# HyeonwooNoh/VQA-Transfer-ExternalData

Measured on AMD Instinct MI355X. Metric: VQA train samples/sec (img+question) at bs512, higher is better.
Workload: dtype f32

## Files before the change

### include/vqa_hot.h

```cpp
#ifndef VQA_HOT_H
#define VQA_HOT_H

#include <stdint.h>

#ifdef __cplusplus
extern "C" {
#endif

#define VQA_HOT_ABI_VERSION 5

enum {
    VQA_OK = 0,
    VQA_ERR_ARG = -1,
    VQA_ERR_ALIGN = -2,
    VQA_ERR_LAUNCH = -3,
    VQA_ERR_UNSUPPORTED = -4,
    VQA_ERR_WORKSPACE = -5
};

int vqa_hot_version(void);
const char* vqa_hot_error_string(int code);

int vqa_gather_features(const float* table, const int32_t* nbox_table, const int64_t* idx,
                        float* V, int32_t* nb, int B, int R, int D, int64_t N, void* stream);

int vqa_embed_fwd(const float* E, const int32_t* q, float* x_tm, int B, int T, int W, int Vq, void* stream);
int vqa_gru_pack_wx(const float* wg, const float* wc, const float* bg, const float* bc, float* wx, float* bx, int W, int H,
                    void* stream);
int vqa_gru_unpack_dwx(const float* dwx, float* gwg, float* gwc, int W, int H, void* stream);
int vqa_embed_fwd_ld(const float* E, const int32_t* q, float* x_tm, int B, int T, int W, int Vq, int ldx, void* stream);
int vqa_gru_unpack_dwx_bias(const float* dwx, float* gwg, float* gwc, float* gbg, float* gbc, int W, int H, void* stream);
int vqa_set_deterministic(int on);
int vqa_embed_bwd(const float* dx_tm, const int32_t* q, float* dE, int B, int T, int W, int Vq, void* stream);
int vqa_embed_bwd_len(const float* dx_tm, const int32_t* q, const int32_t* len, float* dE, int B, int T, int W,
                      int Vq, void* stream);
int vqa_embed_bwd_len_det(const float* dx_tm, const int32_t* q, const int32_t* len, float* dE, int B, int T, int W,
                          int Vq, int deterministic, void* stream);

int vqa_gemm_f32(int transA, int transB, int M, int N, int K, const float* A, int lda, const float* B,
                 int ldb, float* C, int ldc, const float* bias, const float* D, int ldd, int split_k,
                 float* workspace, int64_t workspace_floats, void* stream);
int vqa_gemm_f32_ex(int transA, int transB, int M, int N, int K, const float* A, int lda, const float* B,
                    int ldb, float* C, int ldc, const float* bias, const float* D, int ldd, int split_k,
                    float* workspace, int64_t workspace_floats, int max_blocks, void* stream);
int vqa_gemm_f32_gather(int M, int N, int K, const float* table, int lda, const int64_t* idx, int R,
                        int64_t n_samples_in_table, const float* B, int ldb, float* C, int ldc, const float* bias,
                        float* gathered_out, int ldg, void* stream);
int vqa_gemm_set_max_blocks(int n);
int vqa_gemm_set_order(int order);
int64_t vqa_gemm_workspace_floats(int transA, int transB, int M, int N, int K, int split_k);
int vqa_gemm_set_config(int cfg);
int vqa_gemm_set_gru_config(int cfg);
int vqa_gemm_set_tall_config(int cfg);

int vqa_ln_set_fast(int on);
int vqa_ln_relu_fwd(const float* pre, const float* gamma, const float* beta, const uint8_t* keepmask,
                    float keep_prob, float* y, float* mean, float* rstd, int G, int rows, int N, void* stream);
int vqa_ln_relu_bwd(const float* dy, const float* pre, const float* mean, const float* rstd,
                    const float* gamma, const float* beta, const uint8_t* keepmask, float keep_prob,
                    float* dpre, float* part_dgamma, float* part_dbeta, float* part_dbias, int G, int rows,
                    int N, void* stream);
int vqa_ln_act_fwd(const float* pre, const float* gamma, const float* beta, const uint8_t* keepmask, float keep_prob,
                   float* y, float* mean, float* rstd, int G, int rows, int N, int act, void* stream);
int vqa_ln_act_bwd(const float* dy, const float* pre, const float* mean, const float* rstd, const float* gamma,
                   const float* beta, const uint8_t* keepmask, float keep_prob, float* dpre, float* part_dgamma,
                   float* part_dbeta, float* part_dbias, int G, int rows, int N, int act, void* stream);
int vqa_ln_pair_mul_supported(int N, const void* const* ptrs, int n_ptrs);
int vqa_ln_pair_mul_fwd(const float* pre_a, const float* pre_b, const float* gamma_a, const float* beta_a, const float* gamma_b,
                        const float* beta_b, float* y_a, float* y_b, float* z, float* mean_a, float* rstd_a, float* mean_b,
                        float* rstd_b, int G, int N, void* stream);
int vqa_ln_pair_mul_bwd(const float* dz, const float* add_b, const float* pre_a, const float* pre_b, const float* mean_a,
                        const float* rstd_a, const float* mean_b, const float* rstd_b, const float* gamma_a, const float* beta_a,
                        const float* gamma_b, const float* beta_b, float* dpre_a, float* dpre_b, float* part_dgamma_a,
                        float* part_dbeta_a, float* part_dbias_a, float* part_dgamma_b, float* part_dbeta_b, float* part_dbias_b,
                        int G, int N, void* stream);
int vqa_tanh_fwd(const float* x, float* y, int64_t n, void* stream);
int vqa_tanh_bwd(const float* dy, const float* y, float* dx, int64_t n, void* stream);
int vqa_colsum(const float* X, int M, int N, int ldx, float* out, float* workspace, int64_t workspace_floats,
               void* stream);
int64_t vqa_colsum_workspace_floats(int M, int N);
int vqa_colsum3(const float* X0, const float* X1, const float* X2, int M, int N, int ldx, float* out0, float* out1,
                float* out2, float* workspace, int64_t workspace_floats, void* stream);
int vqa_colsum_acc(const float* X, int M, int N, int ldx, float* out, int accumulate, float* workspace,
                   int64_t workspace_floats, void* stream);
int vqa_colsum3_acc(const float* X0, const float* X1, const float* X2, int M, int N, int ldx, float* out0, float* out1,
                    float* out2, int acc_mask, float* workspace, int64_t workspace_floats, void* stream);
int vqa_mul(const float* a, const float* b, float* z, int64_t n, void* stream);
int vqa_mul_bwd(const float* dz, const float* a, const float* b, float* da, float* db, int64_t n, void* stream);
int vqa_add_inplace(float* acc, const float* x, int64_t n, void* stream);

int vqa_gru_gates_fwd(const float* gpre, int ldg, const float* h_prev, float* r, float* u, float* rh, int B,
                      int H, void* stream);
int vqa_gru_cand_fwd(const float* cpre, int ldc, const float* u, const float* h_prev, const int32_t* len, int t,
                     float* c, float* h_new, int B, int H, void* stream);
int vqa_gru_bwd_a(const float* dh, const float* h_prev, const float* u, const float* c, const int32_t* len,
                  int t, float* dc_pre, int ld_dc, float* du_pre, int ld_du, float* dh_acc, int B, int H,
                  void* stream);
int vqa_gru_bwd_b(const float* drh, const float* h_prev, const float* r, float* dr_pre, int ld_dr,
                  float* dh_acc, int B, int H, void* stream);

int vqa_gru_seq_fwd(float* xp, const float* Wg_h, const float* Wc_h, const int32_t* len, float* hs, float* r,
                    float* u, float* c, float* rh, int T, int B, int H, void* stream);
int vqa_gru_seq_bwd(float* dh_T, const float* Wg_h, const float* Wc_h, const int32_t* len, const float* hs,
                    const float* r, const float* u, const float* c, float* dxp, float* dh_scratch, int T, int B,
                    int H, void* stream);

int vqa_gru_seq_fwd_live(float* xp, const float* Wg_h, const float* Wc_h, const int32_t* len, const int32_t* live_rows,
                         float* hs, float* r, float* u, float* c, float* rh, int T, int B, int H, void* stream);
int vqa_gru_seq_bwd_live(float* dh_T, const float* Wg_h, const float* Wc_h, const int32_t* len,
                         const int32_t* live_rows, const float* hs, const float* r, const float* u, const float* c,
                         float* dxp, float* dh_scratch, int T, int B, int H, void* stream);
int vqa_gru_fill_finished(float* hs, float* rh, const int32_t* len, int T, int B, int H, void* stream);
int vqa_gru_zero_finished(float* dxp, const int32_t* len, int T, int B, int H, void* stream);

int vqa_gru_seq_fwd_persistent(const float* xp, const float* Wg_h, const float* Wc_h, const int32_t* len, float* hs,
                               float* r, float* u, float* c, float* rh, int T, int B, int H, unsigned* sync,
                               void* stream);
int vqa_gru_fwd_persistent_supported(int T, int B, int H);
int64_t vqa_gru_persistent_sync_bytes(void);
int vqa_gru_set_persistent(int mode);
int vqa_gru_persistent_set_census(unsigned* dev_words);

int vqa_gru_seq_fwd_ws(const float* xp, const float* Wg_h, const float* Wc_h, const int32_t* len, float* hs, float* r,
                       float* u, float* c, float* rh, int T, int B, int H, void* ws, void* stream);
int vqa_gru_ws_supported(int T, int B, int H);
int vqa_gru_seq_bwd_ws(const float* dh_T, const float* d_outs, const float* Wg_h, const float* Wc_h, const int32_t* len,
                       const float* hs, const float* r, const float* u, const float* c, float* dxp, int T, int B, int H,
                       void* ws, void* stream);
int vqa_gru_ws_bwd_supported(int T, int B, int H);
int64_t vqa_gru_ws_workspace_bytes(int T);
int vqa_gru_ws_set_mode(int mode);
int vqa_gru_ws_set_form(int form);
int vqa_gru_ws_set_stamps(unsigned long long* dev_words);

int vqa_gru_seq_fwd_rows(float* xp, const float* Wg_h, const float* Wc_h, const int32_t* len, float* hs, float* r,
                         float* u, float* c, float* rh, int T, int B, int H, int row0, int rows, void* stream);
// ... 338 lines not shown
```

### vqa-transfer-externaldata_amd/_lib.py

```python
from __future__ import annotations

import ctypes as C
import os

_HERE = os.path.dirname(os.path.abspath(__file__))
_LIB_PATH = os.path.join(_HERE, "libvqahot.so")


class VqaHotError(RuntimeError):
    pass


def lib_path():
    return _LIB_PATH


class Dims(C.Structure):
    _fields_ = [("B", C.c_int32), ("R", C.c_int32), ("D", C.c_int32), ("H", C.c_int32), ("T", C.c_int32),
                ("W", C.c_int32), ("A", C.c_int32), ("Vq", C.c_int32), ("N_img", C.c_int64),
                ("model_type", C.c_int32), ("keep_att", C.c_float), ("keep_joint", C.c_float),
                ("inv_global_batch", C.c_float), ("flags", C.c_int32),
                ("num_marginal", C.c_int32), ("ent_cols", C.c_int32), ("extra_weight", C.c_float),
                ("map_dim", C.c_int32), ("La", C.c_int32)]

# ... 24 lines not shown
    _fields_ = [("table", C.c_void_p), ("nbox_table", C.c_void_p), ("image_idx", C.c_void_p),
                ("q_intseq", C.c_void_p), ("q_intseq_len", C.c_void_p), ("answer_target", C.c_void_p),
                ("train_mask", C.c_void_p), ("obj_mask", C.c_void_p), ("attr_mask", C.c_void_p),
                ("exist_mask", C.c_void_p), ("keep_att", C.c_void_p), ("keep_joint", C.c_void_p),
                ("keep_joint2", C.c_void_p), ("live_rows", C.c_void_p), ("noise", C.c_void_p), ("keep_tile", C.c_void_p),
                ("keep_word", C.c_void_p), ("answer_intseq", C.c_void_p), ("answer_intseq_len", C.c_void_p)]


class PtDims(C.Structure):
    _fields_ = [(k, C.c_int32) for k in ("B", "n", "R", "D", "H", "W", "A", "Vq", "n_ws", "L", "flags")] + \
               [("keep_att", C.c_float), ("keep_joint", C.c_float), ("global_valid", C.c_float * 2)]


class PtFc(C.Structure):
    _fields_ = [("w", C.c_void_p), ("b", C.c_void_p), ("beta", C.c_void_p * 4), ("gamma", C.c_void_p * 4)]


class PtParams(C.Structure):
    _fields_ = [("wordset_map", C.c_void_p), ("l_glove", C.c_void_p), ("spat_v_linear_v", PtFc),
                ("spat_q_linear_v", PtFc), ("spat_att_score", PtFc), ("gru_wg", C.c_void_p), ("gru_bg", C.c_void_p),
                ("gru_wc", C.c_void_p), ("gru_bc", C.c_void_p), ("pooled_linear_l", PtFc), ("q_linear_l", PtFc),
                ("joint_fc", PtFc), ("wordset_ft", PtFc), ("classifier", PtFc)]


class PtKind(C.Structure):
    _fields_ = [(k, C.c_void_p) for k in ("normal_boxes", "fills", "blanks", "blanks_len", "wordsets", "num", "keep_att",
                                          "keep_bf_joint", "keep_ws_joint")]


class PtBatch(C.Structure):
    _fields_ = [("image_ft", C.c_void_p), ("spatial_ft", C.c_void_p), ("num_boxes", C.c_void_p), ("kind", PtKind * 2),
                ("perm", C.c_void_p), ("inv", C.c_void_p), ("live_rows", C.c_void_p)]


PT_HEAD_BF, PT_HEAD_WS, PT_HEAD_EW = 1, 2, 4


class PtExtDims(C.Structure):
    _fields_ = [("base", PtDims), ("heads", C.c_int32), ("Lc", C.c_int32), ("n_ctx", C.c_int32)]


class PtFc6(C.Structure):
    _fields_ = [("w", C.c_void_p), ("b", C.c_void_p), ("beta", C.c_void_p * 6), ("gamma", C.c_void_p * 6)]


class PtExtParams(C.Structure):
    _fields_ = [("wordset_map", C.c_void_p), ("l_glove", C.c_void_p), ("enwiki_map", C.c_void_p),
                ("spat_v_linear_v", PtFc6), ("spat_q_linear_v", PtFc6), ("spat_att_score", PtFc6)] + \
               [(k, C.c_void_p) for k in ("gru_wg", "gru_bg", "gru_wc", "gru_bc", "egru_wg", "egru_bg", "egru_wc",
                                          "egru_bc")] + \
               [(k, PtFc6) for k in ("pooled_linear_l", "q_linear_l", "joint_fc", "wordset_ft", "classifier")]


class PtCtxKind(C.Structure):
    _fields_ = [(k, C.c_void_p) for k in ("context", "context_len", "keep_ew_joint")]


class PtExtBatch(C.Structure):
    _fields_ = [("base", PtBatch), ("ctx", PtCtxKind * 2), ("ctx_perm", C.c_void_p), ("ctx_inv", C.c_void_p),
                ("ctx_live_rows", C.c_void_p)]


_P, _I, _L, _F = C.c_void_p, C.c_int, C.c_int64, C.c_float

SIGNATURES = {
    "vqa_hot_version": (_I, []),
    "vqa_hot_error_string": (C.c_char_p, [_I]),
    "vqa_gather_features": (_I, [_P, _P, _P, _P, _P, _I, _I, _I, _L, _P]),
    "vqa_embed_fwd": (_I, [_P, _P, _P, _I, _I, _I, _I, _P]),
    "vqa_gru_pack_wx": (_I, [_P, _P, _P, _P, _P, _P, _I, _I, _P]),
    "vqa_gru_unpack_dwx": (_I, [_P, _P, _P, _I, _I, _P]),
    "vqa_embed_fwd_ld": (_I, [_P, _P, _P, _I, _I, _I, _I, _I, _P]),
    "vqa_gru_unpack_dwx_bias": (_I, [_P, _P, _P, _P, _P, _I, _I, _P]),
    "vqa_embed_bwd": (_I, [_P, _P, _P, _I, _I, _I, _I, _P]),
    "vqa_embed_bwd_len": (_I, [_P, _P, _P, _P, _I, _I, _I, _I, _P]),
    "vqa_embed_bwd_len_det": (_I, [_P, _P, _P, _P, _I, _I, _I, _I, _I, _P]),
    "vqa_set_deterministic": (_I, [_I]),
    "vqa_gemm_f32": (_I, [_I, _I, _I, _I, _I, _P, _I, _P, _I, _P, _I, _P, _P, _I, _I, _P, _L, _P]),
    "vqa_gemm_workspace_floats": (_L, [_I, _I, _I, _I, _I, _I]),
    "vqa_gemm_f32_ex": (_I, [_I, _I, _I, _I, _I, _P, _I, _P, _I, _P, _I, _P, _P, _I, _I, _P, _L, _I, _P]),
    "vqa_gemm_f32_gather": (_I, [_I, _I, _I, _P, _I, _P, _I, _L, _P, _I, _P, _I, _P, _P, _I, _P]),
    "vqa_gemm_set_tall_config": (_I, [_I]),
    "vqa_gemm_set_max_blocks": (_I, [_I]),
    "vqa_gemm_set_order": (_I, [_I]),
    "vqa_gemm_set_config": (_I, [_I]),
    "vqa_conv_set_config": (_I, [_I]),
    "vqa_gemm_set_gru_config": (_I, [_I]),
    "vqa_gru_seq_fwd": (_I, [_P, _P, _P, _P, _P, _P, _P, _P, _P, _I, _I, _I, _P]),
    "vqa_gru_seq_fwd_persistent": (_I, [_P, _P, _P, _P, _P, _P, _P, _P, _P, _I, _I, _I, _P, _P]),
    "vqa_gru_fwd_persistent_supported": (_I, [_I, _I, _I]),
    "vqa_gru_persistent_sync_bytes": (_L, []),
    "vqa_gru_set_persistent": (_I, [_I]),
    "vqa_gru_persistent_set_census": (_I, [_P]),
    "vqa_gru_seq_fwd_ws": (_I, [_P, _P, _P, _P, _P, _P, _P, _P, _P, _I, _I, _I, _P, _P]),
    "vqa_gru_ws_supported": (_I, [_I, _I, _I]),
    "vqa_gru_seq_bwd_ws": (_I, [_P, _P, _P, _P, _P, _P, _P, _P, _P, _P, _I, _I, _I, _P, _P]),
    "vqa_gru_ws_bwd_supported": (_I, [_I, _I, _I]),
    "vqa_gru_ws_workspace_bytes": (_L, [_I]),
    "vqa_gru_ws_set_mode": (_I, [_I]),
    "vqa_gru_ws_set_form": (_I, [_I]),
    "vqa_gru_ws_set_stamps": (_I, [_P]),
    "vqa_gru_seq_fwd_rows": (_I, [_P, _P, _P, _P, _P, _P, _P, _P, _P, _I, _I, _I, _I, _I, _P]),
    "vqa_gru_seq_bwd_rows": (_I, [_P, _P, _P, _P, _P, _P, _P, _P, _P, _P, _I, _I, _I, _I, _I, _P]),
    "vqa_gru_seq_bwd": (_I, [_P, _P, _P, _P, _P, _P, _P, _P, _P, _P, _I, _I, _I, _P]),
    "vqa_gru_seq_fwd_live": (_I, [_P, _P, _P, _P, _P, _P, _P, _P, _P, _P, _I, _I, _I, _P]),
    "vqa_gru_seq_bwd_live": (_I, [_P, _P, _P, _P, _P, _P, _P, _P, _P, _P, _P, _I, _I, _I, _P]),
    "vqa_gru_fill_finished": (_I, [_P, _P, _P, _I, _I, _I, _P]),
    "vqa_gru_zero_finished": (_I, [_P, _P, _I, _I, _I, _P]),
    "vqa_ln_set_fast": (_I, [_I]),
    "vqa_ln_relu_fwd": (_I, [_P, _P, _P, _P, _F, _P, _P, _P, _I, _I, _I, _P]),
    "vqa_ln_relu_bwd": (_I, [_P, _P, _P, _P, _P, _P, _P, _F, _P, _P, _P, _P, _I, _I, _I, _P]),
    "vqa_ln_act_fwd": (_I, [_P, _P, _P, _P, _F, _P, _P, _P, _I, _I, _I, _I, _P]),
    "vqa_ln_act_bwd": (_I, [_P, _P, _P, _P, _P, _P, _P, _F, _P, _P, _P, _P, _I, _I, _I, _I, _P]),
    "vqa_ln_pair_mul_supported": (_I, [_I, _P, _I]),
    "vqa_ln_pair_mul_fwd": (_I, [_P] * 13 + [_I, _I, _P]),
    "vqa_ln_pair_mul_bwd": (_I, [_P] * 20 + [_I, _I, _P]),
    "vqa_tanh_fwd": (_I, [_P, _P, _L, _P]),
    "vqa_tanh_bwd": (_I, [_P, _P, _P, _L, _P]),
    "vqa_softmax_ce_fwd": (_I, [_P, _P, _P, _I, _P, _P, _P, _I, _I, _P]),
    "vqa_softmax_set_fast": (_I, [_I]),
    "vqa_colsum": (_I, [_P, _I, _I, _I, _P, _P, _L, _P]),
    "vqa_colsum_workspace_floats": (_L, [_I, _I]),
    "vqa_colsum3": (_I, [_P, _P, _P, _I, _I, _I, _P, _P, _P, _P, _L, _P]),
    "vqa_colsum_acc": (_I, [_P, _I, _I, _I, _P, _I, _P, _L, _P]),
    "vqa_colsum3_acc": (_I, [_P, _P, _P, _I, _I, _I, _P, _P, _P, _I, _P, _L, _P]),
    "vqa_mul": (_I, [_P, _P, _P, _L, _P]),
    "vqa_mul_bwd": (_I, [_P, _P, _P, _P, _P, _L, _P]),
    "vqa_add_inplace": (_I, [_P, _P, _L, _P]),
    "vqa_gru_gates_fwd": (_I, [_P, _I, _P, _P, _P, _P, _I, _I, _P]),
    "vqa_gru_cand_fwd": (_I, [_P, _I, _P, _P, _P, _I, _P, _P, _I, _I, _P]),
    "vqa_gru_bwd_a": (_I, [_P, _P, _P, _P, _P, _I, _P, _I, _P, _I, _P, _I, _I, _P]),
    "vqa_gru_bwd_b": (_I, [_P, _P, _P, _P, _I, _P, _I, _I, _P]),
    "vqa_attn_set_fast": (_I, [_I]),
    "vqa_attn_pool_fwd": (_I, [_P, _P, _P, _P, _P, _P, _P, _F, _P, _P, _I, _I, _I, _I, _P]),
    "vqa_attn_pool_bwd": (_I, [_P, _P, _P, _P, _P, _P, _P, _F, _P, _P, _P, _P, _I, _I, _I, _I, _P]),
    "vqa_attn_pool_fwd_rep": (_I, [_P, _P, _P, _P, _P, _P, _P, _F, _P, _P, _I, _I, _I, _I, _I, _P]),
    "vqa_attn_pool_bwd_rep": (_I, [_P, _P, _P, _P, _P, _P, _P, _F, _P, _P, _P, _P, _I, _I, _I, _I, _I, _P]),
    "vqa_loss_fwd": (_I, [_P, _P, _P, _P, _P, _P, _I, _F, _P, _P, _P, _I, _I, _P]),
    "vqa_loss2_fwd": (_I, [_P, _P, _P, _P, _P, _P, _P, _F, _P, _P, _P, _P, _P, _I, _I, _I, _P]),
    "vqa_rowmin_mask_fwd": (_I, [_P, _P, _P, _P, _I, _I, _P]),
    "vqa_rowmin_mask_bwd": (_I, [_P, _P, _P, _P, _I, _I, _P]),
    "vqa_report_reduce": (_I, [_P, _I, _P, _P]),
    "vqa_report_key": (C.c_char_p, [_I]),
    "vqa_sumsq": (_I, [_P, _L, _P, _P, _P, _L, _P]),
    "vqa_sumsq_workspace_floats": (_L, [_L]),
    "vqa_clip_adam": (_I, [_P, _P, _P, _P, _L, _P, _F, _F, _F, _F, _F, _P]),
    "vqa_dropout_mask": (_I, [_P, _L, C.c_uint64, C.c_uint64, _F, _P]),
    "vqa_clip_adam_dev": (_I, [_P, _P, _P, _P, _L, _P, _F, _P, _F, _F, _F, _P]),
    "vqa_embed2_fwd": (_I, [_P, _P, _P, _P, _I, _I, _I, _I, _P]),
    "vqa_embed2_bwd": (_I, [_P, _P, _P, _P, _I, _I, _I, _I, _P]),
    "vqa_lstm_step_fwd": (_I, [_P, _P, _P, _P, _I, _P, _P, _I, _I, _P]),
    "vqa_lstm_step_bwd": (_I, [_P, _P, _P, _P, _P, _P, _I, _P, _P, _P, _I, _I, _P]),
    "vqa_relu_fwd": (_I, [_P, _P, _L, _P]),
    "vqa_relu_bwd": (_I, [_P, _P, _P, _L, _P]),
    "vqa_fill": (_I, [_P, _L, _F, _P]),
    "vqa_score_fwd": (_I, [_P, _P, _P, _P, _P, _I, _I, _I, _P]),
    "vqa_score_bwd": (_I, [_P, _P, _P, _P, _P, _P, _P, _I, _I, _I, _P]),
    "vqa_reverse_tokens": (_I, [_P, _P, _P, _I, _I, _P]),
    "vqa_bi_outputs_fwd": (_I, [_P, _P, _P, _P, _P, _I, _I, _I, _P]),
    "vqa_bi_outputs_bwd": (_I, [_P, _P, _P, _P, _P, _P, _P, _I, _I, _I, _P]),
    "vqa_bi_dx_combine": (_I, [_P, _P, _P, _P, _I, _I, _I, _P]),
    "vqa_gru_seq_bwd_outs": (_I, [_P, _P, _P, _P, _P, _P, _P, _P, _P, _P, _P, _I, _I, _I, _P]),
    "vqa_adam_lr_step": (_I, [_P, _P, C.c_double, C.c_double, _P, _P]),
    "vqa_graph_capture_begin": (_I, [_P]),
    "vqa_graph_capture_end": (_I, [_P, C.POINTER(C.c_void_p), C.POINTER(C.c_int)]),
    "vqa_graph_capture_abort": (_I, [_P]),
# ... 93 lines not shown
```

### vqa-transfer-externaldata_amd/csrc/gemm_f32.hip

```cpp

#include "vqa_common.h"
#include "gemm_args.h"
#include <cstdio>
#include <cstdlib>

#ifndef VQA_GEMM_STAGGER
#define VQA_GEMM_STAGGER 1
#endif

typedef float f32x16 __attribute__((ext_vector_type(16)));
typedef unsigned int u32x4 __attribute__((ext_vector_type(4)));

#if defined(VQA_DBG_STAMPS)
__device__ unsigned long long* g_dbg_stamps = nullptr;
#define DBG_STAMP(i) do { if (threadIdx.x == 0) dbg_t[i] = __builtin_amdgcn_s_memrealtime(); } while (0)
#else
#define DBG_STAMP(i) do {} while (0)
#endif

namespace {


__device__ __forceinline__ int xcd_remap(int lin, int total) {
    const int q = total >> 3, r = total & 7;
// ... 843 lines not shown
        a.m_fastest = (g_force_order >= 0) ? g_force_order : (m_fast < n_fast ? 1 : 0);
    }
    a.vec_epi = (a.N % 4 == 0) && (a.ldc % 4 == 0) && vqa_aligned16(a.C) && (a.slab_stride % 4 == 0) &&
                (a.D == nullptr || (a.ldd % 4 == 0 && vqa_aligned16(a.D))) &&
                (a.bias == nullptr || vqa_aligned16(a.bias)) && (a.scale == nullptr || vqa_aligned16(a.scale));
    int blocks = a.tiles_m * a.tiles_n * split;
    if (max_blocks > 0 && WGK == 1 && EPI == EPI_PLAIN && blocks > max_blocks) blocks = max_blocks;
    hipLaunchKernelGGL(kern, dim3(blocks), dim3(NT), lds, st, a, ep);
    VQA_CHECK_LAUNCH();
    return VQA_OK;
}

template <int BM, int BN, int WM, int WN, int WGK, int BK, int DEEP, int NT = 256>
int launch_cfg(int tA, int tB, const GemmArgs& a, int split, hipStream_t st, int mb) {
    const EpiArgs ep{};
    if (tA == 0 && tB == 0)
        return launch_one<BM, BN, WM, WN, WGK, BK, DEEP, true, false, EPI_PLAIN, false, false, NT>(a, ep, split, st, mb);
    if (tA == 0 && tB == 1)
        return launch_one<BM, BN, WM, WN, WGK, BK, DEEP, true, true, EPI_PLAIN, false, false, NT>(a, ep, split, st, mb);
    return launch_one<BM, BN, WM, WN, WGK, BK, DEEP, false, false, EPI_PLAIN, false, false, NT>(a, ep, split, st, mb);
}

struct TileCfg { int BM, BN; };
constexpr int NUM_CFG = 24;
const TileCfg kCfg[NUM_CFG] = {{128, 128}, {128, 128}, {64, 64}, {64, 64}, {64, 64}, {128, 64}, {64, 128},
                               {64, 32}, {32, 32}, {32, 64}, {64, 64}, {64, 32}, {64, 64}, {64, 32}, {128, 32},
                               {128, 64}, {128, 128}, {128, 128}, {256, 64}, {128, 128}, {128, 64}, {64, 128}, {128, 64}, {64, 32}};

bool fast_ok(int tA, int tB, GemmArgs& a) {
    if (!a.vecA || !a.vecB || a.K < 4 || (a.K % 4) != 0) return false;
    if (tA && ((a.M % 4) != 0 || a.M < 4)) return false;
    if (!tB && ((a.N % 4) != 0 || a.N < 4)) return false;
    const int64_t ab = (tA ? ((int64_t)(a.K - 1) * a.lda + a.M) : ((int64_t)(a.M - 1) * a.lda + a.K)) * 4;
    const int64_t bb = (tB ? ((int64_t)(a.N - 1) * a.ldb + a.K) : ((int64_t)(a.K - 1) * a.ldb + a.N)) * 4;
    if (ab >= 0xFFFFFF00ll || bb >= 0xFFFFFF00ll) return false;
    a.a_bytes = (unsigned)ab;
    a.b_bytes = (unsigned)bb;
    return true;
}

int launch_edge(int tA, int tB, const GemmArgs& a, int split, hipStream_t st) {
    const EpiArgs ep{};
    if (tA == 0 && tB == 0)
        return launch_one<64, 64, 32, 32, 1, 16, false, true, false, EPI_PLAIN, false, true>(a, ep, split, st, 0);
    if (tA == 0 && tB == 1)
        return launch_one<64, 64, 32, 32, 1, 16, false, true, true, EPI_PLAIN, false, true>(a, ep, split, st, 0);
    return launch_one<64, 64, 32, 32, 1, 16, false, false, false, EPI_PLAIN, false, true>(a, ep, split, st, 0);
}

int launch_by_id(int cfg, int tA, int tB, const GemmArgs& a_in, int split, hipStream_t st, int mb = 0) {
    GemmArgs a = a_in;
    if (!fast_ok(tA, tB, a)) return launch_edge(tA, tB, a, split, st);
    switch (cfg) {
        case 0: return launch_cfg<128, 128, 64, 64, 1, 16, false>(tA, tB, a, split, st, mb);
        case 1: return launch_cfg<128, 128, 64, 64, 1, 32, false>(tA, tB, a, split, st, mb);
        case 2: return launch_cfg<64, 64, 32, 32, 1, 16, false>(tA, tB, a, split, st, mb);
        case 3: return launch_cfg<64, 64, 32, 32, 1, 32, false>(tA, tB, a, split, st, mb);
        case 4: return launch_cfg<64, 64, 32, 32, 1, 64, false>(tA, tB, a, split, st, mb);
        case 5: return launch_cfg<128, 64, 64, 32, 1, 32, false>(tA, tB, a, split, st, mb);
        case 6: return launch_cfg<64, 128, 32, 64, 1, 32, false>(tA, tB, a, split, st, mb);
        case 7: return launch_cfg<64, 32, 32, 32, 2, 64, false>(tA, tB, a, split, st, mb);
        case 8: return launch_cfg<32, 32, 32, 32, 4, 64, false>(tA, tB, a, split, st, mb);
        case 9: return launch_cfg<32, 64, 32, 32, 2, 64, false>(tA, tB, a, split, st, mb);
        case 10: return launch_cfg<64, 64, 32, 32, 1, 64, true>(tA, tB, a, split, st, mb);
        case 11: return launch_cfg<64, 32, 32, 32, 2, 64, true>(tA, tB, a, split, st, mb);
        case 12: return launch_cfg<64, 64, 32, 32, 1, 32, true>(tA, tB, a, split, st, mb);
        case 13: return launch_cfg<64, 32, 32, 32, 2, 32, true>(tA, tB, a, split, st, mb);
        case 14: return launch_cfg<128, 32, 32, 32, 1, 64, true>(tA, tB, a, split, st, mb);
        case 15: return launch_cfg<128, 64, 32, 64, 1, 32, true>(tA, tB, a, split, st, mb);
        case 16: return launch_cfg<128, 128, 64, 32, 1, 32, 0, 512>(tA, tB, a, split, st, mb);
        case 17: return launch_cfg<128, 128, 32, 64, 1, 32, 0, 512>(tA, tB, a, split, st, mb);
        case 18: return launch_cfg<256, 64, 64, 32, 1, 32, 0, 512>(tA, tB, a, split, st, mb);
        case 19: return launch_cfg<128, 128, 64, 32, 1, 16, 0, 512>(tA, tB, a, split, st, mb);
        case 20: return launch_cfg<128, 64, 32, 32, 1, 32, 0, 512>(tA, tB, a, split, st, mb);
        case 21: return launch_cfg<64, 128, 32, 32, 1, 32, 0, 512>(tA, tB, a, split, st, mb);
        case 22: return launch_cfg<128, 64, 32, 32, 1, 16, 0, 512>(tA, tB, a, split, st, mb);
        case 23: return launch_cfg<64, 32, 32, 32, 4, 32, 1, 512>(tA, tB, a, split, st, mb);
        default: return VQA_ERR_ARG;
    }
}

}
int vqa_gru_rs_launch(int epi, const GemmArgs& a, const EpiArgs& ep, hipStream_t st);
namespace {
template <int EPI>
int launch_gru(int cfg, const GemmArgs& a_in, const EpiArgs& ep, hipStream_t st) {
    constexpr bool BKC = (EPI == EPI_BWD_RH || EPI == EPI_BWD_DH);
    GemmArgs a = a_in;
    if (!fast_ok(0, BKC ? 1 : 0, a)) return VQA_ERR_ALIGN;
    if (cfg == 30) {
        const int rc = vqa_gru_rs_launch(EPI, a_in, ep, st);
        if (rc != VQA_ERR_UNSUPPORTED) return rc;
        cfg = 16;
    }
    switch (cfg) {
        case 4: return launch_one<64, 64, 32, 32, 1, 64, false, true, BKC, EPI>(a, ep, 1, st);
        case 7: return launch_one<64, 32, 32, 32, 2, 64, false, true, BKC, EPI>(a, ep, 1, st);
        case 8: return launch_one<32, 32, 32, 32, 4, 64, false, true, BKC, EPI>(a, ep, 1, st);
        case 9: return launch_one<32, 64, 32, 32, 2, 64, false, true, BKC, EPI>(a, ep, 1, st);
        case 10: return launch_one<64, 64, 32, 32, 1, 64, true, true, BKC, EPI>(a, ep, 1, st);
        case 11: return launch_one<64, 32, 32, 32, 2, 64, true, true, BKC, EPI>(a, ep, 1, st);
        case 12: return launch_one<64, 64, 32, 32, 1, 32, true, true, BKC, EPI>(a, ep, 1, st);
        case 13: return launch_one<64, 32, 32, 32, 2, 32, true, true, BKC, EPI>(a, ep, 1, st);
        case 16: return launch_one<32, 32, 32, 32, 4, 32, true, true, BKC, EPI>(a, ep, 1, st);
        case 20: return launch_one<128, 64, 32, 32, 1, 32, 0, true, BKC, EPI, false, false, 512>(a, ep, 1, st);
        case 21: return launch_one<64, 128, 32, 32, 1, 32, 0, true, BKC, EPI, false, false, 512>(a, ep, 1, st);
        case 17: return launch_one<64, 32, 32, 32, 4, 32, 1, true, BKC, EPI, false, false, 512>(a, ep, 1, st);
        case 18:
            if (EPI == EPI_GATES) return launch_one<64, 64, 32, 32, 4, 64, 1, true, BKC, EPI, false, false, 1024>(a, ep, 1, st);
            return launch_one<64, 32, 32, 32, 8, 64, 1, true, BKC, EPI, false, false, 1024>(a, ep, 1, st);
        default: return VQA_ERR_ARG;
    }
}

inline int64_t cdiv(int64_t a, int64_t b) { return (a + b - 1) / b; }

int g_force_cfg = -1;
int g_tall_cfg = 20;
int g_max_blocks = 0;
int g_conv_cfg = -1;
int g_conv_cfg_plain = -1;
int g_gru_cfg = -1;
inline int env_cfg(const char* name, int dflt) {
    const char* e = getenv(name);
    return e ? atoi(e) : dflt;
}
inline int gru_cfg_fwd(int rows) {
    static const int mid = env_cfg("VQA_HOT_GRU_MID_FWD", 9), tall = env_cfg("VQA_HOT_GRU_TALL_FWD", 12);
    return g_gru_cfg >= 0 ? g_gru_cfg : (rows >= 2048 ? tall : rows > 512 ? mid : rows > 256 ? 18 : 16);
}
inline int gru_narrow_override() {
    static const int v = [] { const char* e = getenv("VQA_HOT_GRU_NARROW_CFG"); return e ? atoi(e) : 9; }();
    return v;
}
inline int gru_cfg_fwd_cand(int rows) {
    return (g_gru_cfg < 0 && rows >= 2048 && gru_narrow_override() >= 0) ? gru_narrow_override() : gru_cfg_fwd(rows);
}
inline int gru_cfg_bwd(int rows) {
    static const int mid = env_cfg("VQA_HOT_GRU_MID_BWD", 17), tall = env_cfg("VQA_HOT_GRU_TALL_BWD", 13);
    return g_gru_cfg >= 0 ? g_gru_cfg : (rows >= 2048 ? tall : rows > 512 ? mid : rows > 256 ? 18 : 16);
}

inline int tall_small_cfg() {
    static const int v = [] { const char* e = getenv("VQA_HOT_TALL_SMALL_CFG"); return e ? atoi(e) : 12; }();
    return v < NUM_CFG ? v : 12;
}

inline int tune_pair(const char* env, int cfg, int split) {
    const char* e = getenv(env);
    if (e != nullptr) {
        int c = 0, s = 0;
        if (sscanf(e, "%d:%d", &c, &s) == 2 && c >= 0 && c < NUM_CFG && s >= 0 && s <= 16) { cfg = c; split = s; }
    }
    return (cfg << 8) | split;
}

void choose(int tA, int tB, int M, int N, int K, int& cfg, int& split) {
    int64_t target;
    if (tA) {
        static const int tn_short = env_cfg("VQA_HOT_TN_SHORT_CFG", 20);
        static const int tn_mid = env_cfg("VQA_HOT_TN_MID_CFG", 20);
        const bool mid = K < 20000 && cdiv(M, 128) * cdiv(N, 128) <= 128;
        cfg = ((int64_t)M * N >= (1 << 20)) ? (K <= 4096 ? tn_short : (mid ? tn_mid : 19)) : 3;
        target = 512;
    }
    else if (M >= 2048) {
        cfg = (N >= 512) ? (K >= 2048 ? g_tall_cfg : 22) : 13;
        target = 256;
        if (N >= 512 && cdiv(M, 128) * cdiv(N, 64) < 1024 && tall_small_cfg() >= 0) cfg = tall_small_cfg();
    }
    else { cfg = (!tB && N > 2048) ? 13 : 23; target = 256; }
    int want_split = 0;
    if (!tA && tB && M >= 4096 && N <= 320 && K >= 2048) {
        static const int t = tune_pair("VQA_HOT_DX_TUNE", 3, 4);
        if (t >> 8) { cfg = t >> 8; want_split = t & 255; }
    } else if (tA && M <= 320 && N >= 2048 && K >= 4096) {
        static const int t = tune_pair("VQA_HOT_DWX_TUNE", 21, 4);
        if (t >> 8) { cfg = t >> 8; want_split = t & 255; }
    }
    if (g_force_cfg >= 0 && g_force_cfg < NUM_CFG) { cfg = g_force_cfg; want_split = 0; }
    const int64_t blocks = cdiv(M, kCfg[cfg].BM) * cdiv(N, kCfg[cfg].BN);
    if (split <= 0) {
        split = 1;
        if ((N % 4) == 0) {
            if (want_split > 0) split = want_split;
            else
                while (blocks * split < target && K / (split * 2) >= 256 && split < 16) split *= 2;
        }
    }
}

GemmArgs make_args(int M, int N, int K, const float* A, int lda, const float* B, int ldb, float* C, int ldc,
                   const float* bias, const float* D, int ldd) {
    GemmArgs a;
    a.M = M; a.N = N; a.K = K;
    a.A = A; a.lda = lda; a.B = B; a.ldb = ldb; a.C = C; a.ldc = ldc;
    a.bias = bias; a.D = D; a.ldd = ldd;
    a.vecA = (lda % 4 == 0) && vqa_aligned16(A);
    a.vecB = (ldb % 4 == 0) && vqa_aligned16(B);
    a.slab_stride = 0;
    a.k_per_split = (int)cdiv(std::max(K, 1), 64) * 64;
    a.scale = nullptr; a.relu = 0;
    a.a_bytes = a.b_bytes = 0;
    a.Hi = a.Wi = a.Ci = a.Ho = a.Wo = a.cstride = a.pad_t = a.pad_l = a.kw = a.conv_taps = 0;
    a.g_idx = nullptr; a.g_R = 1; a.g_N = 0; a.g_out = nullptr; a.g_ldo = 0;
    return a;
}

}

extern "C" int64_t vqa_gemm_workspace_floats(int transA, int transB, int M, int N, int K, int split_k) {
    int cfg, split = split_k;
    choose(transA, transB, M, N, K, cfg, split);
    return split > 1 ? (int64_t)split * M * N : 0;
}

extern "C" int vqa_gemm_set_config(int cfg) {
    VQA_REQUIRE(cfg >= -1 && cfg < NUM_CFG, VQA_ERR_ARG);
    g_force_cfg = cfg;
    return VQA_OK;
}

extern "C" int vqa_gemm_set_gru_config(int cfg) {
    VQA_REQUIRE(cfg == -1 || cfg == 4 || (cfg >= 7 && cfg <= 13) || (cfg >= 16 && cfg <= 18) || cfg == 20 || cfg == 21 || cfg == 30,
                VQA_ERR_ARG);
    g_gru_cfg = cfg;
    return VQA_OK;
}

int g_shortk_mode = -1;
inline int shortk_mode() {
    if (g_shortk_mode < 0) {
        const char* e = getenv("VQA_HOT_SHORTK");
        g_shortk_mode = e ? (atoi(e) & 3) : 3;
    }
    return g_shortk_mode;
}
int g_bf16x3_mode = -1;
inline int bf16x3_mode() {
    if (g_bf16x3_mode < 0) {
        const char* e = getenv("VQA_HOT_BF16X3");
        g_bf16x3_mode = (e && atoi(e) != 0) ? 1 : 0;
    }
    return g_bf16x3_mode;
}
extern "C" int vqa_gemm_bf16x3_set_mode(int on) {
    g_bf16x3_mode = on < 0 ? -1 : (on ? 1 : 0);
    return VQA_OK;
}
extern "C" int vqa_gemm_shortk_set_mode(int mode) {
    g_shortk_mode = mode < 0 ? -1 : (mode & 3);
    return VQA_OK;
}

extern "C" int vqa_gemm_f32(int transA, int transB, int M, int N, int K, const float* A, int lda, const float* B,
                            int ldb, float* C, int ldc, const float* bias, const float* D, int ldd, int split_k,
                            float* workspace, int64_t workspace_floats, void* stream) {
    return vqa_gemm_f32_ex(transA, transB, M, N, K, A, lda, B, ldb, C, ldc, bias, D, ldd, split_k, workspace,
                           workspace_floats, g_max_blocks, stream);
}

#if defined(VQA_DBG_STAMPS)
extern "C" int vqa_gemm_dbg_stamps(void* buf) {
    unsigned long long* b = static_cast<unsigned long long*>(buf);
    return hipMemcpyToSymbol(HIP_SYMBOL(g_dbg_stamps), &b, sizeof(b)) == hipSuccess ? VQA_OK : VQA_ERR_LAUNCH;
}
#endif

extern "C" int vqa_gemm_set_order(int order) {
    g_force_order = (order == 0 || order == 1) ? order : -1;
    return VQA_OK;
}

extern "C" int vqa_gemm_set_max_blocks(int n) {
    g_max_blocks = n > 0 ? n : 0;
    return VQA_OK;
}

extern "C" int vqa_gemm_f32_ex(int transA, int transB, int M, int N, int K, const float* A, int lda, const float* B,
                               int ldb, float* C, int ldc, const float* bias, const float* D, int ldd, int split_k,
                               float* workspace, int64_t workspace_floats, int max_blocks, void* stream) {
    VQA_REQUIRE(M >= 0 && N >= 0 && K >= 0, VQA_ERR_ARG);
    if (M == 0 || N == 0) return VQA_OK;
    VQA_REQUIRE(A && B && C, VQA_ERR_ARG);
    VQA_REQUIRE(!(transA == 1 && transB == 1), VQA_ERR_UNSUPPORTED);
    VQA_REQUIRE(lda >= (transA ? M : K) && ldb >= (transB ? K : N) && ldc >= N, VQA_ERR_ARG);
    VQA_REQUIRE(D == nullptr || ldd >= N, VQA_ERR_ARG);
    hipStream_t st = static_cast<hipStream_t>(stream);

    if (bf16x3_mode() && !transB && D == nullptr && max_blocks == 0 && g_force_cfg < 0 && vqa_gemm_bf16x3_supported(M, N, K) &&
        (int64_t)M * N * K >= (1ll << 32) && lda % 4 == 0 && ldb % 4 == 0 && vqa_aligned16(A) && vqa_aligned16(B)) {
        const int tiles = (M / 128) * (N / 128);
        int sp = 1;
        while (tiles * sp < 256 && K / (sp * 2) >= 512 && sp < 16) sp *= 2;
        while (sp > 1 && (workspace == nullptr || workspace_floats < (int64_t)sp * M * N || ldc % 4 != 0 || !vqa_aligned16(C))) sp /= 2;
        return vqa_gemm_bf16x3(transA, M, N, K, A, lda, B, ldb, C, ldc, bias, sp, workspace, workspace_floats, stream);
    }
    if (!transA && !transB && split_k <= 1 && max_blocks == 0 && g_force_cfg < 0 && (shortk_mode() & 1) &&
        M >= 1024 && K <= 304 && vqa_gemm_shortk_supported(M, N, K, lda, ldb, ldc) && !(K > 256 && D != nullptr) && vqa_aligned16(A) &&
        vqa_aligned16(B))
        return vqa_gemm_shortk_nn(M, N, K, A, lda, B, ldb, C, ldc, bias, nullptr, D, ldd, 0, stream);

    int cfg, split = split_k;
    choose(transA, transB, M, N, K, cfg, split);
    if (split > 1 && ((N % 4) != 0 || workspace == nullptr)) split = 1;

    GemmArgs a = make_args(M, N, K, A, lda, B, ldb, C, ldc, bias, D, ldd);
    if (split > 1) {
        VQA_REQUIRE(workspace_floats >= (int64_t)split * M * N, VQA_ERR_WORKSPACE);
        int kps = (int)cdiv(cdiv(K, split), 64) * 64;
        a.k_per_split = kps;
        split = (int)cdiv(K, kps);
    }
    if (split > 1) {
        a.C = workspace; a.ldc = N; a.slab_stride = (int64_t)M * N;
        int rc = launch_by_id(cfg, transA, transB, a, split, st, max_blocks);
        if (rc != VQA_OK) return rc;
        const int64_t n4 = (int64_t)M * N / 4;
        const int grid = (int)std::min<int64_t>(cdiv(n4, 256), 2048);
        hipLaunchKernelGGL(splitk_reduce_kernel, dim3(grid), dim3(256), 0, st, workspace, C, M, N, ldc, split);
        VQA_CHECK_LAUNCH();
        return VQA_OK;
    }
    a.k_per_split = (int)cdiv(std::max(K, 1), 64) * 64;
    return launch_by_id(cfg, transA, transB, a, 1, st, max_blocks);
}

extern "C" int vqa_gemm_f32_gather(int M, int N, int K, const float* table, int lda, const int64_t* idx, int R,
                                   int64_t n_samples_in_table, const float* B, int ldb, float* C, int ldc,
                                   const float* bias, float* gathered_out, int ldg, void* stream) {
    VQA_REQUIRE(M >= 0 && N >= 0 && K > 0 && R > 0 && n_samples_in_table > 0, VQA_ERR_ARG);
    if (M == 0 || N == 0) return VQA_OK;
    VQA_REQUIRE(table && idx && B && C, VQA_ERR_ARG);
    VQA_REQUIRE(lda >= K && ldb >= N && ldc >= N && (gathered_out == nullptr || ldg >= K), VQA_ERR_ARG);
    VQA_REQUIRE(K % 32 == 0 && N % 4 == 0, VQA_ERR_UNSUPPORTED);
    VQA_REQUIRE(lda % 4 == 0 && vqa_aligned16(table) && ldb % 4 == 0 && vqa_aligned16(B) &&
                    (gathered_out == nullptr || (ldg % 4 == 0 && vqa_aligned16(gathered_out))),
                VQA_ERR_ALIGN);
    GemmArgs a = make_args(M, N, K, table, lda, B, ldb, C, ldc, bias, nullptr, 0);
    const int64_t bb = ((int64_t)(K - 1) * ldb + N) * 4;
    VQA_REQUIRE(bb < 0xFFFFFF00ll, VQA_ERR_UNSUPPORTED);
    a.a_bytes = 0;
    a.b_bytes = (unsigned)bb;
    VQA_REQUIRE(gathered_out == nullptr || ((int64_t)(M - 1) * ldg + K) * 4 < 0xFFFFFF00ll, VQA_ERR_UNSUPPORTED);
    a.g_idx = idx; a.g_R = R; a.g_N = n_samples_in_table; a.g_out = gathered_out; a.g_ldo = ldg;
    a.k_per_split = (int)cdiv(K, 64) * 64;
    const EpiArgs ep{};
    hipStream_t st = static_cast<hipStream_t>(stream);
    if (g_tall_cfg == 21)
        return launch_one<64, 128, 32, 32, 1, 32, 0, true, false, EPI_PLAIN, false, false, 512, true>(a, ep, 1, st, 0);
    return launch_one<128, 64, 32, 32, 1, 32, 0, true, false, EPI_PLAIN, false, false, 512, true>(a, ep, 1, st, 0);
}

extern "C" int vqa_gemm_set_tall_config(int cfg) {
    VQA_REQUIRE(cfg == 20 || cfg == 21, VQA_ERR_ARG);
    g_tall_cfg = cfg;
    return VQA_OK;
}

extern "C" int vqa_gru_seq_fwd(float* xp, const float* Wg_h, const float* Wc_h, const int32_t* len, float* hs,
                               float* r, float* u, float* c, float* rh, int T, int B, int H, void* stream) {
    return vqa_gru_seq_fwd_rows(xp, Wg_h, Wc_h, len, hs, r, u, c, rh, T, B, H, 0, B, stream);
}

extern "C" int vqa_gru_seq_fwd_rows(float* xp, const float* Wg_h, const float* Wc_h, const int32_t* len, float* hs,
                                    float* r, float* u, float* c, float* rh, int T, int B, int H, int row0, int rows,
                                    void* stream) {
    VQA_REQUIRE(xp && Wg_h && Wc_h && len && hs && r && u && c && rh && T >= 0 && B > 0 && H > 0, VQA_ERR_ARG);
    VQA_REQUIRE(row0 >= 0 && rows >= 0 && row0 + rows <= B, VQA_ERR_ARG);
    VQA_REQUIRE(H % 4 == 0, VQA_ERR_ALIGN);
    if (rows == 0) return VQA_OK;
    hipStream_t st = static_cast<hipStream_t>(stream);
    const int64_t BH = (int64_t)B * H, o = (int64_t)row0 * H;
    for (int t = 0; t < T; ++t) {
        float* xpt = xp + ((int64_t)t * B + row0) * 3 * H;
        const float* hp = hs + t * BH + o;
        EpiArgs eg{};
        eg.H = H; eg.h_prev = hp; eg.o0 = r + t * BH + o; eg.o1 = u + t * BH + o; eg.o2 = rh + t * BH + o;
        GemmArgs ag = make_args(rows, 2 * H, H, hp, H, Wg_h, 2 * H, nullptr, 0, nullptr, xpt, 3 * H);
        int rc = launch_gru<EPI_GATES>(gru_cfg_fwd(rows), ag, eg, st);
        if (rc != VQA_OK) return rc;
        EpiArgs ec{};
        ec.H = H; ec.t = t; ec.len = len + row0; ec.h_prev = hp; ec.i0 = u + t * BH + o; ec.o0 = c + t * BH + o;
        ec.o1 = hs + (t + 1) * BH + o;
        GemmArgs ac = make_args(rows, H, H, rh + t * BH + o, H, Wc_h, H, nullptr, 0, nullptr, xpt + 2 * H, 3 * H);
        rc = launch_gru<EPI_CAND>(gru_cfg_fwd_cand(rows), ac, ec, st);
        if (rc != VQA_OK) return rc;
    }
    return VQA_OK;
}

extern "C" int vqa_gru_seq_fwd_live(float* xp, const float* Wg_h, const float* Wc_h, const int32_t* len,
                                    const int32_t* live_rows, float* hs, float* r, float* u, float* c, float* rh,
                                    int T, int B, int H, void* stream) {
    VQA_REQUIRE(xp && Wg_h && Wc_h && len && live_rows && hs && r && u && c && rh && T >= 0 && B > 0 && H > 0, VQA_ERR_ARG);
// ... 223 lines not shown
```

Measured before the change: 159,500.

## Add batch-sized GEMM kernel with intra-block K split and LDS reduction

Adds a new 512-thread, 64xBN tile GEMM kernel. Its waves split the K dimension inside the block and reduce partial sums through LDS, so no split-K workspace pass or separate reduce kernel is needed. It is routed by default for specific shapes: config 23 with M of 256 to 512 and N up to 1024, and transA split-2 config 20 cases. The aim is to raise per-tile parallelism for mid-sized batch GEMMs and drop the extra reduction launch. The trade-off is one block per CU with heavy LDS use, plus a new code path whose numerics differ in summation order.

After: 160,100 (median of 6 runs). No clear change (+0.4%).

```diff
diff --git a/include/vqa_hot.h b/include/vqa_hot.h
--- a/include/vqa_hot.h
+++ b/include/vqa_hot.h
@@ -52,6 +52,7 @@
 int vqa_gemm_set_config(int cfg);
 int vqa_gemm_set_gru_config(int cfg);
 int vqa_gemm_set_tall_config(int cfg);
+int vqa_gemm_batch_set_mode(int mode);
 
 int vqa_ln_set_fast(int on);
 int vqa_ln_relu_fwd(const float* pre, const float* gamma, const float* beta, const uint8_t* keepmask,
diff --git a/vqa-transfer-externaldata_amd/_lib.py b/vqa-transfer-externaldata_amd/_lib.py
--- a/vqa-transfer-externaldata_amd/_lib.py
+++ b/vqa-transfer-externaldata_amd/_lib.py
@@ -130,6 +130,7 @@
     "vqa_gemm_f32_gather": (_I, [_I, _I, _I, _P, _I, _P, _I, _L, _P, _I, _P, _I, _P, _P, _I, _P]),
     "vqa_gemm_set_tall_config": (_I, [_I]),
     "vqa_gemm_set_max_blocks": (_I, [_I]),
+    "vqa_gemm_batch_set_mode": (_I, [_I]),
     "vqa_gemm_set_order": (_I, [_I]),
     "vqa_gemm_set_config": (_I, [_I]),
     "vqa_conv_set_config": (_I, [_I]),
diff --git a/vqa-transfer-externaldata_amd/csrc/gemm_batch.hip b/vqa-transfer-externaldata_amd/csrc/gemm_batch.hip
--- /dev/null
+++ b/vqa-transfer-externaldata_amd/csrc/gemm_batch.hip
@@ -0,0 +1,280 @@
+
+#include "vqa_common.h"
+#include "gemm_args.h"
+
+namespace {
+
+typedef float f32x16 __attribute__((ext_vector_type(16)));
+typedef unsigned int u32x4 __attribute__((ext_vector_type(4)));
+
+constexpr int BM = 64;
+constexpr int NT = 512;
+constexpr unsigned OOB = 0xFFFFFFF0u;
+
+__device__ __forceinline__ int xcd_remap(int lin, int total) {
+    const int q = total >> 3, r = total & 7;
+    const int xcd = lin & 7, idx = lin >> 3;
+    return (xcd < r ? xcd * (q + 1) : r * (q + 1) + (xcd - r) * q) + idx;
+}
+
+__device__ __forceinline__ float4 as_f4(u32x4 v) {
+    return make_float4(__uint_as_float(v.x), __uint_as_float(v.y), __uint_as_float(v.z), __uint_as_float(v.w));
+}
+
+template <int BR, int DEPTH, bool KC, bool HALVES>
+struct Tile {
+    static constexpr int LD = DEPTH + 4;
+    static constexpr int FL = KC ? BR * LD : DEPTH * BR;
+    static constexpr int QPR = KC ? DEPTH / 4 : BR / 4;
+    static constexpr int NV = BR * DEPTH / 4 / NT;
+    static_assert(NV * NT == BR * DEPTH / 4, "whole float4 per thread");
+    unsigned off[NV];
+    u32x4 reg[NV];
+
+    __device__ __forceinline__ void init(int ld, int r0, int RLIM, int kadd) {
+#pragma unroll
+        for (int i = 0; i < NV; ++i) {
+            const int idx = threadIdx.x + i * NT;
+            const int a = idx / QPR, q = (idx % QPR) * 4;
+            if (KC) {
+                const int k = (HALVES && q >= DEPTH / 2) ? q + kadd : q;
+                off[i] = (unsigned)(((int64_t)min(r0 + a, RLIM - 1) * ld + k) * 4);
+            } else {
+                const int k = (HALVES && a >= DEPTH / 2) ? a + kadd : a;
+                off[i] = (unsigned)(((int64_t)k * ld + (r0 + q < RLIM ? r0 + q : 0)) * 4);
+            }
+        }
+    }
+    __device__ __forceinline__ void load(__amdgpu_buffer_rsrc_t rs, unsigned soff) {
+#pragma unroll
+        for (int i = 0; i < NV; ++i) reg[i] = __builtin_amdgcn_raw_buffer_load_b128(rs, off[i], soff, 0);
+    }
+    __device__ __forceinline__ void load_tail(__amdgpu_buffer_rsrc_t rs, int ld, int k0, int K) {
+#pragma unroll
+        for (int i = 0; i < NV; ++i) {
+            const int idx = threadIdx.x + i * NT;
+            const int a = idx / QPR, q = (idx % QPR) * 4;
+            const int k = k0 + (KC ? q : a);
+            const unsigned kb = (unsigned)(KC ? k0 : k0 * ld) * 4u;
+            reg[i] = __builtin_amdgcn_raw_buffer_load_b128(rs, k < K ? off[i] + kb : OOB, 0, 0);
+        }
+    }
+    __device__ __forceinline__ void store(float* s) const {
+#pragma unroll
+        for (int i = 0; i < NV; ++i) {
+            const int idx = threadIdx.x + i * NT;
+            const int a = idx / QPR, q = (idx % QPR) * 4;
+            *reinterpret_cast<float4*>(s + a * (KC ? LD : BR) + q) = as_f4(reg[i]);
+        }
+    }
+};
+
+template <int BR, int DEPTH, bool KC>
+__device__ __forceinline__ float4 frag4(const float* s, int r0, int c, int lane) {
+    const int i = lane & 31, h = lane >> 5;
+    if (KC) return *reinterpret_cast<const float4*>(s + (r0 + i) * (DEPTH + 4) + c * 8 + h * 4);
+    const float* p = s + (c * 8 + h * 4) * BR + r0 + i;
+    return make_float4(p[0], p[BR], p[2 * BR], p[3 * BR]);
+}
+
+template <bool HALVES>
+struct Form {
+    static constexpr int TN = HALVES ? 2 : 1;
+    static constexpr int BN = 32 * TN;
+    static constexpr int G = HALVES ? 2 : 4;
+    static constexpr int SUB = 8 / G;
+    static constexpr int SUB_N = SUB / 2;
+    static constexpr int TW = TN / SUB_N;
+    static constexpr int DEPTH = 128;
+    static constexpr int STEP = HALVES ? DEPTH / 2 : DEPTH;
+    static constexpr int NC = DEPTH / 8 / G;
+};
+
+template <bool HALVES, bool A_KC, bool B_KC>
+constexpr size_t lds_bytes() {
+    using F = Form<HALVES>;
+    const size_t a = A_KC ? BM * (F::DEPTH + 4) : F::DEPTH * BM, b = B_KC ? F::BN * (F::DEPTH + 4) : F::DEPTH * F::BN;
+    const size_t ops = 2 * (a + b), red = (size_t)F::G * BM * (F::BN + 4);
+    return (ops > red ? ops : red) * sizeof(float);
+}
+
+template <bool HALVES, bool A_KC, bool B_KC>
+__global__ __launch_bounds__(NT, 1) void gemm_batch_kernel(GemmArgs p) {
+    using F = Form<HALVES>;
+    constexpr int BN = F::BN, G = F::G, SUB = F::SUB, TW = F::TW, DEPTH = F::DEPTH, NC = F::NC;
+    using TA = Tile<BM, DEPTH, A_KC, HALVES>;
+    using TB = Tile<BN, DEPTH, B_KC, HALVES>;
+    extern __shared__ __attribute__((aligned(16))) float smem[];
+    float* const L0 = smem;
+    float* const L1 = smem + TA::FL + TB::FL;
+
+    const int lane = threadIdx.x & 63, wave = threadIdx.x >> 6;
+    const int sub = wave % SUB, g = wave / SUB;
+    const int wr = (sub & 1) * 32, wc = (sub >> 1) * TW * 32;
+    const int tile = xcd_remap(blockIdx.x, p.tiles_m * p.tiles_n);
+    const int m0 = (tile % p.tiles_m) * BM, n0 = (tile / p.tiles_m) * BN;
+
+    f32x16 acc[TW];
+#pragma unroll
+    for (int b = 0; b < TW; ++b)
+#pragma unroll
+        for (int r = 0; r < 16; ++r) acc[b][r] = 0.f;
+
+    const __amdgpu_buffer_rsrc_t rsA = __builtin_amdgcn_make_buffer_rsrc(const_cast<float*>(p.A), 0, (int)p.a_bytes, 0x00020000);
+    const __amdgpu_buffer_rsrc_t rsB = __builtin_amdgcn_make_buffer_rsrc(const_cast<float*>(p.B), 0, (int)p.b_bytes, 0x00020000);
+    const int kadd = p.k_per_split - F::STEP;
+    TA sa;
+    TB sb;
+    sa.init(p.lda, m0, p.M, kadd);
+    sb.init(p.ldb, n0, p.N, kadd);
+    const unsigned stepA = (unsigned)(A_KC ? F::STEP : F::STEP * p.lda) * 4u;
+    const unsigned stepB = (unsigned)(B_KC ? F::STEP : F::STEP * p.ldb) * 4u;
+    const int nfull = HALVES ? p.k_per_split / F::STEP : p.K / DEPTH;
+    const int nt = HALVES ? nfull : nfull + (p.K % DEPTH != 0);
+    auto fetch = [&](int t) {
+        if (HALVES || t < nfull) {
+            sa.load(rsA, (unsigned)t * stepA);
+            sb.load(rsB, (unsigned)t * stepB);
+        } else {
+            sa.load_tail(rsA, p.lda, t * DEPTH, p.K);
+            sb.load_tail(rsB, p.ldb, t * DEPTH, p.K);
+        }
+    };
+    auto chunk = [&](int cc) { return HALVES ? g * NC + cc : cc * G + g; };
+    auto compute = [&](const float* As, const float* Bs) {
+        float4 af[2], bf[2][TW];
+        af[0] = frag4<BM, DEPTH, A_KC>(As, wr, chunk(0), lane);
+#pragma unroll
+        for (int b = 0; b < TW; ++b) bf[0][b] = frag4<BN, DEPTH, B_KC>(Bs, wc + b * 32, chunk(0), lane);
+#pragma unroll
+        for (int cc = 0; cc < NC; ++cc) {
+            const int cur = cc & 1, nx = cur ^ 1;
+            if (cc + 1 < NC) {
+                af[nx] = frag4<BM, DEPTH, A_KC>(As, wr, chunk(cc + 1), lane);
+#pragma unroll
+                for (int b = 0; b < TW; ++b) bf[nx][b] = frag4<BN, DEPTH, B_KC>(Bs, wc + b * 32, chunk(cc + 1), lane);
+            }
+            __builtin_amdgcn_sched_barrier(0);
+#pragma unroll
+            for (int j = 0; j < 4; ++j)
+#pragma unroll
+                for (int b = 0; b < TW; ++b) {
+                    const float x = j == 0 ? af[cur].x : j == 1 ? af[cur].y : j == 2 ? af[cur].z : af[cur].w;
+                    const float y = j == 0 ? bf[cur][b].x : j == 1 ? bf[cur][b].y : j == 2 ? bf[cur][b].z : bf[cur][b].w;
+                    acc[b] = __builtin_amdgcn_mfma_f32_32x32x2f32(x, y, acc[b], 0, 0, 0);
+                }
+            __builtin_amdgcn_sched_barrier(0);
+        }
+    };
+    auto step = [&](int t, float* cur, float* nxt) {
+        const bool more = t + 1 < nt;
+        if (more) fetch(t + 1);
+        __builtin_amdgcn_sched_barrier(0);
+        compute(cur, cur + TA::FL);
+        __builtin_amdgcn_sched_barrier(0);
+        if (more) {
+            sa.store(nxt);
+            sb.store(nxt + TA::FL);
+        }
+        __syncthreads();
+    };
+
+    if (nt > 0) {
+        fetch(0);
+        sa.store(L0);
+        sb.store(L0 + TA::FL);
+    }
+    __syncthreads();
+    int t = 0;
+    for (; t + 1 < nt; t += 2) {
+        step(t, L0, L1);
+        step(t + 1, L1, L0);
+    }
+    if (t < nt) step(t, L0, L1);
+
+    constexpr int SLD = BN + 4;
+    constexpr int Q = BN / 4;
+    constexpr int RPW = BM / 8;
+    constexpr int ITEMS = RPW * Q / 64;
+    static_assert(ITEMS * 64 == RPW * Q, "whole float4 per lane");
+    float4 bv[ITEMS], dv[ITEMS];
+#pragma unroll
+    for (int i = 0; i < ITEMS; ++i) {
+        const int idx = lane + 64 * i;
+        const int grow = m0 + wave * RPW + idx / Q, gcol = n0 + (idx % Q) * 4;
+        const bool ok = grow < p.M && gcol < p.N;
+        bv[i] = (ok && p.bias != nullptr) ? *reinterpret_cast<const float4*>(p.bias + gcol) : make_float4(0.f, 0.f, 0.f, 0.f);
+        dv[i] = (ok && p.D != nullptr) ? *reinterpret_cast<const float4*>(p.D + (int64_t)grow * p.ldd + gcol)
+                                       : make_float4(0.f, 0.f, 0.f, 0.f);
+    }
+    float* part = smem + g * BM * SLD;
+#pragma unroll
+    for (int b = 0; b < TW; ++b)
+#pragma unroll
+        for (int r = 0; r < 16; ++r)
+            part[(wr + (r & 3) + 8 * (r >> 2) + 4 * (lane >> 5)) * SLD + wc + b * 32 + (lane & 31)] = acc[b][r];
+    __syncthreads();
+#pragma unroll
+    for (int i = 0; i < ITEMS; ++i) {
+        const int idx = lane + 64 * i;
+        const int row = wave * RPW + idx / Q, c4 = (idx % Q) * 4;
+        const int grow = m0 + row, gcol = n0 + c4;
+        const float* src = smem + row * SLD + c4;
+        const float4 s0 = *reinterpret_cast<const float4*>(src);
+        float4 o;
+        if (HALVES) {
+            float4 s1 = *reinterpret_cast<const float4*>(src + BM * SLD);
+            s1.x += 0.f; s1.y += 0.f; s1.z += 0.f; s1.w += 0.f;
+            o = make_float4(s0.x + bv[i].x + dv[i].x + s1.x, s0.y + bv[i].y + dv[i].y + s1.y,
+                            s0.z + bv[i].z + dv[i].z + s1.z, s0.w + bv[i].w + dv[i].w + s1.w);
+        } else {
+            float4 s = s0;
+#pragma unroll
+            for (int q = 1; q < G; ++q) {
+                const float4 v = *reinterpret_cast<const float4*>(src + q * BM * SLD);
+                s.x += v.x; s.y += v.y; s.z += v.z; s.w += v.w;
+            }
+            o = make_float4(s.x + bv[i].x + dv[i].x, s.y + bv[i].y + dv[i].y, s.z + bv[i].z + dv[i].z,
+                            s.w + bv[i].w + dv[i].w);
+        }
+        if (grow < p.M && gcol < p.N) *reinterpret_cast<float4*>(p.C + (int64_t)grow * p.ldc + gcol) = o;
+    }
+}
+
+template <bool HALVES, bool A_KC, bool B_KC>
+int launch(GemmArgs a, hipStream_t st) {
+    constexpr size_t lds = lds_bytes<HALVES, A_KC, B_KC>();
+    auto kern = gemm_batch_kernel<HALVES, A_KC, B_KC>;
+    static bool attr_done = false;
+    if (!attr_done) {
+        if (hipFuncSetAttribute(reinterpret_cast<const void*>(kern), hipFuncAttributeMaxDynamicSharedMemorySize,
+                                (int)lds) != hipSuccess)
+            return VQA_ERR_LAUNCH;
+        attr_done = true;
+    }
+    a.tiles_m = (a.M + BM - 1) / BM;
+    a.tiles_n = (a.N + Form<HALVES>::BN - 1) / Form<HALVES>::BN;
+    hipLaunchKernelGGL(kern, dim3(a.tiles_m * a.tiles_n), dim3(NT), lds, st, a);
+    VQA_CHECK_LAUNCH();
+    return VQA_OK;
+}
+
+template <bool HALVES>
+int launch_layout(int tA, int tB, const GemmArgs& a, hipStream_t st) {
+    if (tA) return launch<HALVES, false, false>(a, st);
+    if (tB) return launch<HALVES, true, true>(a, st);
+    return launch<HALVES, true, false>(a, st);
+}
+
+}
+
+int vqa_gemm_batch_launch(int tA, int tB, const GemmArgs& a, int halves, hipStream_t st) {
+    if (a.N % 4 != 0 || a.ldc % 4 != 0 || !vqa_aligned16(a.C) || (a.bias != nullptr && !vqa_aligned16(a.bias)) ||
+        (a.D != nullptr && (a.ldd % 4 != 0 || !vqa_aligned16(a.D))) || a.K < 4)
+        return VQA_ERR_UNSUPPORTED;
+    if (halves) {
+        if (a.K != 2 * a.k_per_split || a.k_per_split % Form<true>::STEP != 0) return VQA_ERR_UNSUPPORTED;
+        return launch_layout<true>(tA, tB, a, st);
+    }
+    return launch_layout<false>(tA, tB, a, st);
+}
diff --git a/vqa-transfer-externaldata_amd/csrc/gemm_f32.hip b/vqa-transfer-externaldata_amd/csrc/gemm_f32.hip
--- a/vqa-transfer-externaldata_amd/csrc/gemm_f32.hip
+++ b/vqa-transfer-externaldata_amd/csrc/gemm_f32.hip
@@ -949,6 +949,7 @@
 
 }
 int vqa_gru_rs_launch(int epi, const GemmArgs& a, const EpiArgs& ep, hipStream_t st);
+int vqa_gemm_batch_launch(int tA, int tB, const GemmArgs& a, int halves, hipStream_t st);
 namespace {
 template <int EPI>
 int launch_gru(int cfg, const GemmArgs& a_in, const EpiArgs& ep, hipStream_t st) {
@@ -1111,6 +1112,18 @@
     }
     return g_bf16x3_mode;
 }
+int g_batch_mode = -1;
+inline int batch_mode() {
+    if (g_batch_mode < 0) {
+        const char* e = getenv("VQA_HOT_BATCH_GEMM");
+        g_batch_mode = e ? (atoi(e) & 3) : 1;
+    }
+    return g_batch_mode;
+}
+extern "C" int vqa_gemm_batch_set_mode(int mode) {
+    g_batch_mode = mode < 0 ? -1 : (mode & 3);
+    return VQA_OK;
+}
 extern "C" int vqa_gemm_bf16x3_set_mode(int on) {
     g_bf16x3_mode = on < 0 ? -1 : (on ? 1 : 0);
     return VQA_OK;
@@ -1178,6 +1191,19 @@
         int kps = (int)cdiv(cdiv(K, split), 64) * 64;
         a.k_per_split = kps;
         split = (int)cdiv(K, kps);
+    }
+    if (batch_mode() && max_blocks == 0 && g_force_cfg < 0) {
+        const bool halves = split == 2 && K == 2 * a.k_per_split;
+        const bool routed = halves ? (transA && cfg == 20 && (int64_t)M * N <= (1 << 20))
+                                   : (split == 1 && cfg == 23 && M >= 256 && M <= 512 && N <= 1024);
+        if (routed || batch_mode() == 2) {
+            GemmArgs b = a;
+            if (split == 1) b.k_per_split = (int)cdiv(std::max(K, 1), 64) * 64;
+            if ((split == 1 || halves) && fast_ok(transA, transB, b)) {
+                const int rc = vqa_gemm_batch_launch(transA, transB, b, halves ? 1 : 0, st);
+                if (rc != VQA_ERR_UNSUPPORTED) return rc;
+            }
+        }
     }
     if (split > 1) {
         a.C = workspace; a.ldc = N; a.slab_stride = (int64_t)M * N;
```
